# ZhangT-tech/MoCA-Video

Measured on AMD Instinct MI355X. Metric: denoising UNet-steps/sec @16x320x512 fp16, higher is better.
Workload: dtype f16

## Files before the change

### include/moca_hip.h

```cpp
#ifndef MOCA_HIP_H
#define MOCA_HIP_H

#include <stdint.h>

#ifdef __cplusplus
extern "C" {
#endif

#define MOCA_OK            0
#define MOCA_E_BADARG     -1
#define MOCA_E_LAUNCH     -2
#define MOCA_E_NODEVICE   -3
#define MOCA_E_GRAPH      -4

#define MOCA_A_LINEAR   0
#define MOCA_A_CONV3X3  1
#define MOCA_A_TCONV3   2

#define MOCA_EP_GEGLU   1
#define MOCA_EP_OUT_F32 2
#define MOCA_FORCE_SMALL_TILE 4
#define MOCA_EP_COLSUM 16
#define MOCA_EP_LN     32
#define MOCA_EP_GELU    8
// ... 181 lines not shown
    const float* coef;
    const int32_t* win_start;
    const float* mask;
    const float* mask_sums;
    const int32_t* mask_frame;
    const float* enh;
    const float* cond;
    const float* sam_eff;
    const int32_t* sam_idx;
    float cfg_scale, beta, one_minus_beta, gamma, one_minus_gamma;
    int32_t nW, C, Q, f, HW, wb_from;
} moca_fifo_step_params;
int moca_fifo_step_windows_f32(const moca_fifo_step_params* p, void* stream);
int moca_sam_select_masks_f32(const float* cand, const int32_t* cand_off, const int32_t* ncand, const int64_t* t_rows, float* eff,
                              int32_t* eff_idx, int32_t nW, int32_t f, int32_t HW, void* stream);
int moca_fifo_advance_f32(moca_fifo_state* state, float* queue, const float* newframe, float* emitted, int32_t n_slots,
                          int32_t emit_frame, float* mask, float* mask_sums, int32_t C, int32_t Q, int32_t HW, void* stream);
int moca_fifo_prepare_queue_f32(const float* z, const float* noise, float* queue, const float* coef_z, const float* coef_noise,
                                const int32_t* frame_idx, int32_t BC, int32_t Tz, int32_t Q, int32_t HW, void* stream);
int moca_base_set_timestep(const moca_fifo_state* state, const int64_t* table, int32_t S, int64_t* rows, int32_t n, void* stream);
int moca_base_ddim_step_f32(moca_fifo_state* state, float* x, const float* eps_c, const float* eps_u, const float* noise,
                            float* pred_x0, const float* coef, int32_t S, float cfg_scale, int32_t use_scale, int64_t n, void* stream);
int moca_mask_frame_sums_f32(const float* mask, float* sums, int32_t frames, int32_t HW, void* stream);

int moca_freq_mix_3d_f32(const float* x, const float* noise, const float* lpf, float* out,
                         int32_t C, int32_t T, int32_t H, int32_t W, float* ws, void* stream);
int64_t moca_freq_mix_ws_bytes(int32_t C, int32_t T, int32_t H, int32_t W);
int moca_freq_filter_f32(float* lpf, int32_t T, int32_t H, int32_t W, int32_t type, int32_t n,
                         double d_s, double d_t, void* stream);

int moca_graph_begin(void* stream);
int moca_graph_end(void* stream, void** graph_exec_out);
int moca_graph_launch(void* graph_exec, void* stream);
int moca_graph_destroy(void* graph_exec);
int moca_stream_create(void** stream_out);
int moca_stream_destroy(void* stream);
int moca_stream_sync(void* stream);
int moca_event_create(void** ev_out);
int moca_event_record(void* ev, void* stream);
int moca_event_elapsed_ms(void* ev_start, void* ev_stop, float* ms_out);
int moca_event_destroy(void* ev);

#define MOCA_TUNE_GEMM_W80   0
#define MOCA_TUNE_GEMM_G4    1
#define MOCA_TUNE_GEMM_SQ256 2
#define MOCA_TUNE_GEMM_WIDE  3
#define MOCA_TUNE_GN_SLAB    4
#define MOCA_TUNE_GEMM_G4P   5
#define MOCA_TUNE_GEMM_MF32  6
#define MOCA_TUNE_GEMM_SQP   7
#define MOCA_TUNE_SQP_WALK   8
#define MOCA_TUNE_SLAB_F16   9
#define MOCA_TUNE_GEMM_WS    10
#define MOCA_TUNE_COUNT      11
int moca_set_tuning(int32_t knob, int32_t value);
int moca_debug_clock_sampler(void* buf, int32_t blocks, int32_t nsamples, const int32_t* stop, void* stream);

int moca_device_info(char* name, int32_t len, int32_t* cu_count);
const char* moca_version(void);

#ifdef __cplusplus
}
#endif
#endif
```

### moca_video_amd/csrc/gemm.hip

```cpp
#include "common.h"

namespace {

template <int V> struct int_c { static constexpr int value = V; };
struct yes_t { static constexpr bool value = true; };
struct no_t { static constexpr bool value = false; };

constexpr int BM = 128;
constexpr int BK = 64;
constexpr int MOCA_A_LINEAR2 = 3;
constexpr int ROW_BYTES = BK * 2;

struct Geo {
    int C, inH, inW, outH, outW, stride, up, T, HW;
};

__device__ __forceinline__ void remap_tile_2d(int tiles_m, int tiles_n, int xn, int& tile_m, int& tile_n) {
    const int xm = 8 / xn;
    const int sm = tiles_m / xm, sn = tiles_n / xn;
    const int b = blockIdx.x;
    const int xcd = b & 7, j = b >> 3;
    const int xi = xcd / xn, xj = xcd - xi * xn;
    tile_m = xi * sm + j / sn;
    tile_n = xj * sn + j % sn;
// ... 2537 lines not shown
            float sum = 0.f;
#pragma unroll
            for (int r = 0; r < 4; ++r) {
                const float pv = exp2f((sc[i][r] - mx) * sl2e);
                sum += pv;
                pf[i][r] = (half_t)pv;
            }
            sum = xlane16_sum(sum);
            sum = xlane32_sum(sum);
            inv[i] = 1.0f / sum;
        }
#pragma unroll
        for (int i = 0; i < NPX; ++i) {
            half_t* ob = outp + (int64_t)grow(pixs[i] * 16 + fr) * p.ldo + tile_n * 64;
            const bool live = wave + 8 * i < 20;
#pragma unroll
            for (int dt = 0; dt < 4; ++dt) {
                f32x4 o4 = {0.f, 0.f, 0.f, 0.f};
                o4 = __builtin_amdgcn_mfma_f32_16x16x16f16(vfr[i][dt], pf[i], o4, 0, 0, 0);
                half4v h4;
#pragma unroll
                for (int r = 0; r < 4; ++r) h4[r] = (half_t)(o4[r] * inv[i]);
                if (live) *reinterpret_cast<half4v*>(ob + dt * 16 + 4 * fg) = h4;
            }
        }
    } else if constexpr (SQ) {
        store_fp16_tile<512>(p, smem, pitch, TM, BN, m0, n0, tid);
    } else if constexpr (WIDE) {
        if (p.flags & MOCA_EP_LN) store_fp16_tile_ln(p, smem, reinterpret_cast<float*>(smem + TM * pitch), pitch, m0, tid);
        else if (p.flags & (MOCA_EP_COLSUM | MOCA_EP_GSTAT)) store_fp16_tile_colsum<TM, BN>(p, smem, reinterpret_cast<float*>(smem + TM * pitch), pitch, m0, n0, tile_m, tid);
        else if (p.flags & MOCA_EP_ROWSUM) store_fp16_tile_rowsum<512, BN, 8>(p, smem, pitch, TM, m0, n0, tid);
        else store_fp16_tile<512>(p, smem, pitch, TM, BN, m0, n0, tid);
    } else {
        if (p.flags & (MOCA_EP_COLSUM | MOCA_EP_GSTAT)) store_fp16_tile_colsum<TM, BN>(p, smem, reinterpret_cast<float*>(smem + TM * pitch), pitch, m0, n0, tile_m, tid);
        else if (p.flags & MOCA_EP_ROWSUM) store_fp16_tile_rowsum<512, BN, 4>(p, smem, pitch, TM, m0, n0, tid);
        else store_fp16_tile<512>(p, smem, pitch, TM, BN, m0, n0, tid);
    }
    MOCA_STAMP(5);
    MOCA_STAMP_HW();
#endif
}

__device__ __forceinline__ void lds_wr_f2(unsigned a, f32x2 v) { asm volatile("ds_write_b64 %0, %1" ::"v"(a), "v"(v) : "memory"); }
__device__ __forceinline__ void lds_wr_f1(unsigned a, float v) { asm volatile("ds_write_b32 %0, %1" ::"v"(a), "v"(v) : "memory"); }
__device__ __forceinline__ f32x2 lds_rd_f2(unsigned a) { f32x2 v; asm volatile("ds_read_b64 %0, %1" : "=v"(v) : "v"(a) : "memory"); return v; }
__device__ __forceinline__ f32x4 lds_rd_f4(unsigned a) { f32x4 v; asm volatile("ds_read_b128 %0, %1" : "=v"(v) : "v"(a) : "memory"); return v; }
__device__ __forceinline__ float lds_rd_f1(unsigned a) { float v; asm volatile("ds_read_b32 %0, %1" : "=v"(v) : "v"(a) : "memory"); return v; }
__device__ __forceinline__ void lds_wait() { asm volatile("s_waitcnt lgkmcnt(0)" ::: "memory"); __builtin_amdgcn_sched_barrier(0); }

__device__ __forceinline__ int sqp_perm(int rho) {
    return (rho & ~63) + (g4p_perm(rho & 127) & 63);
}

template <bool GEGLU>
__global__ __launch_bounds__(512, 2) void gemm_sqp_kernel(const moca_gemm_params p) {
#if defined(__HIP_DEVICE_COMPILE__)
#ifndef SEG_WAVE
#define SEG_WAVE 0
#endif
    constexpr int MT = 4, NT = 8, KS = 32, RB = 64, WTM = 64, WTN = 128, TM = 256, BN = 256;
    constexpr int A_BYTES = TM * RB, STAGE = A_BYTES + BN * RB, NS = 5, PPW = 4;
    extern __shared__ __attribute__((aligned(16))) char smem[];

    const int tid = threadIdx.x, lane = tid & 63;
    const int wave = __builtin_amdgcn_readfirstlane(tid >> 6);
    const int wave_m = wave >> 1, wave_n = wave & 1;
    const bool late = wave >= 4;
    const int nper = p.reserved2_;
    if (prefetch_block(p, nper, 512)) return;

    const int tiles_n = p.N / BN, tiles_m = (p.M + TM - 1) / TM;
    const int xcd_n = p.reserved4_ >> 8;
    const int J = nper >> 3;
    int q_base, q_cnt, sub_n, tm_base, tn_base;
    {
        const int x = blockIdx.x & 7;
        if (xcd_n > 1) {
            const int xm = 8 / xcd_n, sm = tiles_m / xm;
            sub_n = tiles_n / xcd_n;
            const int xi = x / xcd_n, xj = x - xi * xcd_n;
            tm_base = xi * sm; tn_base = xj * sub_n;
            q_base = 0; q_cnt = sm * sub_n;
        } else {
            const int ntiles = tiles_m * tiles_n, q = ntiles >> 3, r = ntiles & 7;
            q_base = x < r ? x * (q + 1) : r * (q + 1) + (x - r) * q;
            q_cnt = q + (x < r ? 1 : 0);
            sub_n = tiles_n; tm_base = 0; tn_base = 0;
        }
    }
    auto tile_of = [&](int q, int& tm, int& tn) {
        const int l = q_base + q;
        const int a = l / sub_n;
        tm = tm_base + a; tn = tn_base + (l - a * sub_n);
    };
    int q_cur, q_step, q_end;
    {
        const int j = blockIdx.x >> 3;
        if (p.reserved4_ & 2) {
            q_cur = (int)((int64_t)q_cnt * j / J);
            q_end = (int)((int64_t)q_cnt * (j + 1) / J);
            q_step = 1;
        } else {
            q_cur = j; q_end = q_cnt; q_step = J;
        }
    }
    if (q_cur >= q_end) return;
    const int nk = p.K / 32;

    const int lrow = lane >> 2, pch = lane & 3;
    const int lch = pch ^ ((0x78 >> (2 * ((lrow >> 2) & 3))) & 3);
    const __amdgpu_buffer_rsrc_t rsrc_a = __builtin_amdgcn_make_buffer_rsrc(const_cast<void*>(p.a), 0, OOB_OFF, 0x00020000);
    const __amdgpu_buffer_rsrc_t rsrc_w = __builtin_amdgcn_make_buffer_rsrc(const_cast<void*>(p.w), 0, OOB_OFF, 0x00020000);
    unsigned a_off[2], w_off[2];
    int d_q = q_cur, d_k = 0;
    auto set_dma_tile = [&](int q) {
        int tm, tn;
        tile_of(q, tm, tn);
        const bool any = q < q_end;
#pragma unroll
        for (int g = 0; g < 2; ++g) {
            const int row = tm * TM + (g * 8 + wave) * 16 + lrow;
            a_off[g] = (any && row < p.M) ? (unsigned)(((int64_t)row * p.lda + lch * 8) * 2) : OOB_OFF;
            w_off[g] = any ? (unsigned)(((int64_t)(tn * BN + sqp_perm((g * 8 + wave) * 16 + lrow)) * p.ldw + lch * 8) * 2) : OOB_OFF;
        }
    };
    auto issue_pair = [&](int slot_even, int slot_odd) {
        const unsigned soff = (unsigned)(d_k * KS * 2);
        const lds_ptr se = (lds_ptr)smem + slot_even * STAGE, so = (lds_ptr)smem + slot_odd * STAGE;
#pragma unroll
        for (int g = 0; g < 2; ++g) {
            __builtin_amdgcn_raw_ptr_buffer_load_lds(rsrc_a, se + (g * 8 + wave) * 1024, 16, a_off[g], soff, 0, 0);
            __builtin_amdgcn_raw_ptr_buffer_load_lds(rsrc_a, so + (g * 8 + wave) * 1024, 16, a_off[g], soff + KS * 2, 0, 0);
        }
#pragma unroll
        for (int g = 0; g < 2; ++g) {
            __builtin_amdgcn_raw_ptr_buffer_load_lds(rsrc_w, se + A_BYTES + (g * 8 + wave) * 1024, 16, w_off[g], soff, 0, 0);
            __builtin_amdgcn_raw_ptr_buffer_load_lds(rsrc_w, so + A_BYTES + (g * 8 + wave) * 1024, 16, w_off[g], soff + KS * 2, 0, 0);
        }
        d_k += 2;
        if (d_k >= nk) { d_k = 0; d_q += q_step; set_dma_tile(d_q); }
    };

    const int fr = lane & 15, fg = lane >> 4;
    const int swz = (fg ^ ((0x78 >> (2 * ((fr >> 2) & 3))) & 3)) << 4;
    const int a_off0 = (wave_m * WTM + fr) * RB + swz;
    const int b_off0 = A_BYTES + (wave_n * WTN + fr) * RB + swz;
    f32x4 acc[MT][NT];
    half8v af[2][MT], bf[2][NT];
    auto read_tile = [&](auto set_tag, int slot) {
        constexpr int S = decltype(set_tag)::value;
        const char* cur = smem + slot * STAGE;
#pragma unroll
        for (int r = 0; r < NT; ++r) bf[S][r] = *reinterpret_cast<const half8v*>(cur + b_off0 + r * 1024);
#pragma unroll
        for (int r = 0; r < MT; ++r) af[S][r] = *reinterpret_cast<const half8v*>(cur + a_off0 + r * 1024);
    };

    auto tid_now = [&]() -> int {
        int l;
        asm volatile("v_mbcnt_lo_u32_b32 %0, -1, 0\n\tv_mbcnt_hi_u32_b32 %0, -1, %0" : "=v"(l));
        return wave * 64 + l;
    };
    const bool fold = (p.flags & MOCA_EP_LNFOLD) != 0;
    const float* const dummy = reinterpret_cast<const float*>(p.w);
    constexpr unsigned STAT_SCRATCH = 8192;
    const int stat_floats = 2 + 2 * (fold ? p.lnf_nparts : 0);
    auto stat_dma = [&](int q, unsigned slot_off) {
        int tm, tn;
        tile_of(q < q_end ? q : 0, tm, tn);
        const int t = tid_now();
        const int n = tn * BN + sqp_perm(t);
        const int m = min(tm * TM + t, p.M - 1);
        const lds_ptr area = (lds_ptr)smem + slot_off + STAT_SCRATCH + wave * (22 * 256);
        __builtin_amdgcn_global_load_lds((glb_ptr)(fold ? p.lnf_wsum + n : dummy), area, 4, 0, 0);
        __builtin_amdgcn_global_load_lds((glb_ptr)(p.bias ? p.bias + n : dummy), area + 256, 4, 0, 0);
        if (fold) {
            for (int i = 0; i < p.lnf_nparts; ++i) {
                const float* src = p.lnf_part + ((int64_t)i * p.M + m) * 2;
                __builtin_amdgcn_global_load_lds((glb_ptr)src, area + (2 + 2 * i) * 256, 4, 0, 0);
                __builtin_amdgcn_global_load_lds((glb_ptr)(src + 1), area + (3 + 2 * i) * 256, 4, 0, 0);
            }
        }
    };
    auto stat_read = [&](unsigned slot_off, auto after_tag) -> LnFoldRegs {
        constexpr int after = decltype(after_tag)::value;
        asm volatile("s_waitcnt vmcnt(%0)" ::"n"(after) : "memory");
        __builtin_amdgcn_sched_barrier(0);
        int lane_;
        asm volatile("v_mbcnt_lo_u32_b32 %0, -1, 0\n\tv_mbcnt_hi_u32_b32 %0, -1, %0" : "=v"(lane_));
        const unsigned area = (unsigned)(size_t)((lds_ptr)smem + slot_off + STAT_SCRATCH + wave * (22 * 256)) + 4 * lane_;
        const float ws = lds_rd_f1(area), b = lds_rd_f1(area + 256);
        float s = 0.f, qq = 0.f;
        LnFoldRegs f = {1.f, 0.f, 0.f, 0.f};
        if (fold) {
            for (int i = 0; i < p.lnf_nparts; ++i) {
                const float x = lds_rd_f1(area + (2 + 2 * i) * 256), y = lds_rd_f1(area + (3 + 2 * i) * 256);
                lds_wait();
                s += x; qq += y;
            }
// ... 18 lines not shown
        lf = stat_read((NS - 1) * STAGE, int_c<0>{});
    }
    __builtin_amdgcn_s_barrier();
    set_dma_tile(q_cur);
    issue_pair(0, 1);
    issue_pair(2, 3);
    asm volatile("s_waitcnt vmcnt(%0)" ::"n"(2 * PPW) : "memory");
    __builtin_amdgcn_s_barrier();
    if (late) __builtin_amdgcn_s_barrier();

    const bool nt_out = out_streams(p);
    const half_t* __restrict__ resid = reinterpret_cast<const half_t*>(p.residual);
    const half_t* __restrict__ rowadd = reinterpret_cast<const half_t*>(p.rowadd);
    int s0 = 0;
#ifdef MOCA_STAMPS
    int tile_no = 0;
#endif
    while (true) {
        int tm, tn;
        tile_of(q_cur, tm, tn);
        const int m0 = tm * TM, n0 = tn * BN;
#ifdef MOCA_STAMPS
        const bool stamp_it = tile_no == 3;
        if (stamp_it) { MOCA_STAMP(0); }
#endif
#pragma unroll
        for (int mt = 0; mt < MT; ++mt)
#pragma unroll
            for (int nt = 0; nt < NT; ++nt) acc[mt][nt] = f32x4{0.f, 0.f, 0.f, 0.f};
        for (int i = 0; i < nk; i += 2) {
            const int s1 = s0 + 1 == NS ? 0 : s0 + 1;
            const int sp = s0 == 0 ? NS - 1 : s0 - 1;
#ifdef MOCA_STAMPS
            const bool seg = stamp_it && i == SEG_ITER;
            if (seg) MOCA_STAMP_W(8, SEG_WAVE);
#endif
            read_tile(int_c<0>{}, s0);
            asm volatile("s_waitcnt lgkmcnt(0)" ::: "memory");
            __builtin_amdgcn_sched_barrier(0);
#ifdef MOCA_STAMPS
            if (seg) MOCA_STAMP_W(9, SEG_WAVE);
#endif
            __builtin_amdgcn_s_barrier();
#ifdef MOCA_STAMPS
            if (seg) MOCA_STAMP_W(10, SEG_WAVE);
#endif
            {
                const char* nx = smem + s1 * STAGE;
                __builtin_amdgcn_s_setprio(1);
#pragma unroll
                for (int j = 0; j < MT * NT; ++j) {
                    const int mt = j / NT, nt = j % NT;
                    acc[mt][nt] = __builtin_amdgcn_mfma_f32_16x16x32_f16(bf[0][nt], af[0][mt], acc[mt][nt], 0, 0, 0);
                    if (j % 2 == 0 && j / 2 < MT + NT) {
                        const int r = j / 2;
                        __builtin_amdgcn_sched_barrier(0);
                        if (r < NT) bf[1][r] = *reinterpret_cast<const half8v*>(nx + b_off0 + r * 1024);
                        else af[1][r - NT] = *reinterpret_cast<const half8v*>(nx + a_off0 + (r - NT) * 1024);
                        __builtin_amdgcn_sched_barrier(0);
                    }
                }
                __builtin_amdgcn_s_setprio(0);
            }
            asm volatile("s_waitcnt lgkmcnt(0)" ::: "memory");
            __builtin_amdgcn_sched_barrier(0);
#ifdef MOCA_STAMPS
            if (seg) MOCA_STAMP_W(11, SEG_WAVE);
#endif
            __builtin_amdgcn_s_barrier();
#ifdef MOCA_STAMPS
            if (seg) MOCA_STAMP_W(12, SEG_WAVE);
#endif
            issue_pair(sp, s0);
#ifdef MOCA_STAMPS
            if (seg) MOCA_STAMP_W(13, SEG_WAVE);
#endif
            asm volatile("s_waitcnt vmcnt(%0)" ::"n"(2 * PPW) : "memory");
            __builtin_amdgcn_sched_barrier(0);
#ifdef MOCA_STAMPS
            if (seg) MOCA_STAMP_W(14, SEG_WAVE);
#endif
            __builtin_amdgcn_s_barrier();
#ifdef MOCA_STAMPS
            if (seg) MOCA_STAMP_W(15, SEG_WAVE);
#endif
            __builtin_amdgcn_s_setprio(1);
#pragma unroll
            for (int mt = 0; mt < MT; ++mt)
#pragma unroll
                for (int nt = 0; nt < NT; ++nt)
                    acc[mt][nt] = __builtin_amdgcn_mfma_f32_16x16x32_f16(bf[1][nt], af[1][mt], acc[mt][nt], 0, 0, 0);
            __builtin_amdgcn_s_setprio(0);
            __builtin_amdgcn_sched_barrier(0);
#ifdef MOCA_STAMPS
            if (seg) MOCA_STAMP_W(1, SEG_WAVE);
#endif
            __builtin_amdgcn_s_barrier();
#ifdef MOCA_STAMPS
            if (seg) MOCA_STAMP_W(2, SEG_WAVE);
#endif
            s0 = s1 + 1 == NS ? 0 : s1 + 1;
        }
#ifdef MOCA_STAMPS
        if (stamp_it) MOCA_STAMP(3);
#endif
        if (!late) __builtin_amdgcn_s_barrier();
        const unsigned lst = (unsigned)(size_t)((lds_ptr)smem + (s0 == 0 ? NS - 1 : s0 - 1) * STAGE);
        const unsigned lws = lst + 8 * TM, lbi = lws + 4 * BN;
        if (!late) {
            const int t = tid_now();
            lds_wr_f2(lst + 8 * t, f32x2{lf.rs, lf.rb});
            lds_wr_f1(lws + 4 * t, lf.ws);
            lds_wr_f1(lbi + 4 * t, lf.b);
        }
        lds_wait();
        __builtin_amdgcn_s_barrier();
#ifdef MOCA_STAMPS
        if (stamp_it) MOCA_STAMP(4);
#endif
        f32x2 st[MT];
#pragma unroll
        for (int mt = 0; mt < MT; ++mt) st[mt] = lds_rd_f2(lst + 8 * (wave_m * WTM + mt * 16 + fr));
        const int q_next = q_cur + q_step;
        const unsigned stat_slot = (unsigned)((s0 == 0 ? NS - 1 : s0 - 1) * STAGE);
        if (!late) stat_dma(q_next, stat_slot);
#pragma unroll
        for (int grp = 0; grp < 2; ++grp) {
            f32x4 cw[4], cb[4];
#pragma unroll
            for (int t = 0; t < 4; ++t) {
                cw[t] = lds_rd_f4(lws + 4 * (wave_n * WTN + (grp * 4 + t) * 16 + 4 * fg));
                cb[t] = lds_rd_f4(lbi + 4 * (wave_n * WTN + (grp * 4 + t) * 16 + 4 * fg));
            }
            lds_wait();
#pragma unroll
            for (int mt = 0; mt < MT; ++mt) {
                const int m = m0 + wave_m * WTM + mt * 16 + fr;
                f32x4 v[4];
#pragma unroll
                for (int t = 0; t < 4; ++t) v[t] = st[mt][0] * acc[mt][grp * 4 + t] + (st[mt][1] * cw[t] + cb[t]);
                if constexpr (GEGLU) {
                    half8v h;
#pragma unroll
                    for (int nv = 0; nv < 2; ++nv) {
                        const f32x4 r4 = moca_geglu4(v[nv], v[nv + 2]);
                        h[4 * nv + 0] = (half_t)r4[0]; h[4 * nv + 1] = (half_t)r4[1]; h[4 * nv + 2] = (half_t)r4[2]; h[4 * nv + 3] = (half_t)r4[3];
                    }
                    if (m < p.M) st_out8(reinterpret_cast<half_t*>(p.out) + (int64_t)m * p.ldo + (n0 >> 1) + wave_n * 64 + grp * 32 + 8 * fg, h, nt_out);
                } else {
#pragma unroll
                    for (int hh = 0; hh < 2; ++hh) {
                        const int col = n0 + wave_n * WTN + grp * 64 + hh * 32 + 8 * fg;
                        float o[8];
#pragma unroll
                        for (int r = 0; r < 4; ++r) { o[r] = v[2 * hh][r]; o[4 + r] = v[2 * hh + 1][r]; }
                        if (m < p.M) {
                            if (rowadd) {
                                const half8v e = *reinterpret_cast<const half8v*>(rowadd + (int64_t)(m / p.rowadd_div) * p.ld_rowadd + col);
#pragma unroll
                                for (int r = 0; r < 8; ++r) o[r] = (float)(half_t)o[r] + (float)e[r];
                            }
                            if (resid) {
                                const half8v e = *reinterpret_cast<const half8v*>(resid + (int64_t)m * p.ldr + col);
#pragma unroll
                                for (int r = 0; r < 8; ++r) o[r] = (rowadd ? o[r] : (float)(half_t)o[r]) + (float)e[r];
                            }
                            half8v h;
#pragma unroll
                            for (int r = 0; r < 8; ++r) h[r] = (half_t)o[r];
                            st_out8(reinterpret_cast<half_t*>(p.out) + (int64_t)m * p.ldo + col, h, nt_out);
                        }
                    }
                }
            }
        }
#ifdef MOCA_STAMPS
        if (stamp_it) { MOCA_STAMP(5); MOCA_STAMP_HW(); }
        ++tile_no;
#endif
        if (!late) {
            if (m0 + TM > p.M) lf = stat_read(stat_slot, int_c<0>{});
            else lf = stat_read(stat_slot, int_c<(GEGLU ? 8 : 16)>{});
        }
        if (q_next >= q_end) break;
        q_cur = q_next;
        if (late) __builtin_amdgcn_s_barrier();
    }
    asm volatile("s_waitcnt vmcnt(0) lgkmcnt(0)" ::: "memory");
#endif
}

static int choose_xcd_n(const moca_gemm_params& p, int tiles_m, int tiles_n, int TM, int BN) {
    if (p.splits != 1 || p.a_mode != MOCA_A_LINEAR) return 1;
    const double Wtot = (double)p.N * p.K * 2, Atot = (double)p.M * p.K * 2;
    auto cost = [&](int xn) {
        const int xm = 8 / xn;
        const double wsub = (double)(tiles_n / xn) * BN * p.K * 2;
        return (wsub <= 3.6e6 ? xm * Wtot : tiles_m * Wtot) + xn * Atot;
    };
    double best = cost(1);
    int best_xn = 1;
    for (int xn = 2; xn <= 8; xn *= 2) {
        if (tiles_m % (8 / xn) || tiles_n % xn) continue;
        const double c = cost(xn);
        if (c < 0.8 * best) { best = c; best_xn = xn; }
    }
    (void)TM;
    return best_xn;
}

template <int AMODE, int SHAPE>
int launch_gemm_w80s(const moca_gemm_params& p, hipStream_t st) {
    constexpr int TM = SHAPE == 2 ? 256 : (SHAPE == 1 ? 160 : 320), BN = SHAPE == 2 ? 256 : (SHAPE == 1 ? 320 : (SHAPE == 3 ? 192 : 160));
    const int tiles_m = (p.M + TM - 1) / TM, tiles_n = p.N / BN;
    const int nblk = tiles_m * tiles_n * p.splits;
    moca_gemm_params pl = p;
    pl.reserved4_ = (pl.reserved4_ & 0xff) | ((SHAPE == 3 ? 1 : choose_xcd_n(p, tiles_m, tiles_n, TM, BN)) << 8);
    constexpr int lds = 5 * (TM + BN) * 64;
    static bool attr_set = false;
    if (!attr_set) {
        if (hipFuncSetAttribute(reinterpret_cast<const void*>(&gemm_w80s_kernel<AMODE, SHAPE>), hipFuncAttributeMaxDynamicSharedMemorySize, lds) != hipSuccess)
            return MOCA_E_LAUNCH;
        attr_set = true;
    }
    hipLaunchKernelGGL((gemm_w80s_kernel<AMODE, SHAPE>), dim3(nblk + prefetch_blocks(pl)), dim3(512), lds, st, pl);
    MOCA_CHECK_LAUNCH();
    return MOCA_OK;
}

static inline int64_t a_span_bytes(const moca_gemm_params& p) {
    if (p.a_mode == MOCA_A_LINEAR) return ((int64_t)p.M * p.lda + 64) * 2;
    if (p.a_mode == MOCA_A_CONV3X3) return ((int64_t)(p.M / (p.outH * p.outW)) * p.inH * p.inW * p.C + 64) * 2;
    return ((int64_t)p.M * p.C + 64) * 2;
}
static inline bool buffer_addressable(const moca_gemm_params& p) {
    if (p.a2 && ((int64_t)p.M * p.lda2 + 64) * 2 >= (1ll << 31)) return false;
    return a_span_bytes(p) < (1ll << 31) && (int64_t)p.N * p.ldw * 2 < (1ll << 31);
}

static inline int sq256_mode() { return moca_tuning_get(MOCA_TUNE_GEMM_SQ256); }
static inline bool fast_gather(const moca_gemm_params& p);
// ... 78 lines not shown
}

constexpr int G4P_BLOCKS = 512;
static inline bool g4p_ok(const moca_gemm_params& p) {
    if (p.a_mode != MOCA_A_LINEAR || p.splits != 1 || p.N % 128 || p.K % 64 || !buffer_addressable(p)) return false;
    if (p.flags & ~(MOCA_EP_GEGLU | MOCA_EP_LNFOLD)) return false;
    if ((p.flags & MOCA_EP_GEGLU) && (p.residual || p.rowadd)) return false;
    return ((p.M + 255) / 256) * (p.N / 128) >= G4P_BLOCKS;
}
template <bool GEGLU>
int launch_gemm_g4p(const moca_gemm_params& p, hipStream_t st) {
    constexpr int lds = 3 * (256 + 128) * 64 + (2 * 256 + 2 * 128) * 4;
    static bool attr_set = false;
    if (!attr_set) {
        if (hipFuncSetAttribute(reinterpret_cast<const void*>(&gemm_g4p_kernel<GEGLU>), hipFuncAttributeMaxDynamicSharedMemorySize, lds) != hipSuccess)
            return MOCA_E_LAUNCH;
        attr_set = true;
    }
    moca_gemm_params pl = p;
    pl.reserved2_ = G4P_BLOCKS;
    if (moca_tuning_get(MOCA_TUNE_GEMM_MF32)) {
        static bool attr_set_q = false;
        if (!attr_set_q) {
            if (hipFuncSetAttribute(reinterpret_cast<const void*>(&gemm_g4q_kernel<GEGLU>), hipFuncAttributeMaxDynamicSharedMemorySize, lds) != hipSuccess)
                return MOCA_E_LAUNCH;
            attr_set_q = true;
        }
        hipLaunchKernelGGL((gemm_g4q_kernel<GEGLU>), dim3(G4P_BLOCKS + 2 * prefetch_blocks(pl)), dim3(256), lds, st, pl);
    } else {
        hipLaunchKernelGGL((gemm_g4p_kernel<GEGLU>), dim3(G4P_BLOCKS + 2 * prefetch_blocks(pl)), dim3(256), lds, st, pl);
    }
    MOCA_CHECK_LAUNCH();
    return MOCA_OK;
}

constexpr int SQP_BLOCKS = 256;
static inline bool sqp_ok(const moca_gemm_params& p) {
    if (p.a_mode != MOCA_A_LINEAR || p.splits != 1 || p.N % 256 || p.K % 64 || !buffer_addressable(p)) return false;
    if (p.flags & ~(MOCA_EP_GEGLU | MOCA_EP_LNFOLD)) return false;
    if ((p.flags & MOCA_EP_GEGLU) && (p.residual || p.rowadd)) return false;
    return ((p.M + 255) / 256) * (p.N / 256) >= SQP_BLOCKS;
}
template <bool GEGLU>
int launch_gemm_sqp(const moca_gemm_params& p, hipStream_t st) {
    constexpr int lds = 5 * (256 + 256) * 64;
    static bool attr_set = false;
    if (!attr_set) {
        if (hipFuncSetAttribute(reinterpret_cast<const void*>(&gemm_sqp_kernel<GEGLU>), hipFuncAttributeMaxDynamicSharedMemorySize, lds) != hipSuccess)
            return MOCA_E_LAUNCH;
        attr_set = true;
    }
    moca_gemm_params pl = p;
    pl.reserved2_ = SQP_BLOCKS;
    pl.reserved4_ = (pl.reserved4_ & 0xfd) | (choose_xcd_n(p, (p.M + 255) / 256, p.N / 256, 256, 256) << 8) |
                    (moca_tuning_get(MOCA_TUNE_SQP_WALK) ? 2 : 0);
    hipLaunchKernelGGL((gemm_sqp_kernel<GEGLU>), dim3(SQP_BLOCKS + prefetch_blocks(pl)), dim3(512), lds, st, pl);
    MOCA_CHECK_LAUNCH();
    return MOCA_OK;
}

template <int BN, int AMODE, bool FAST>
int launch_gemm_glds(const moca_gemm_params& p, hipStream_t st) {
    const int tiles_m = (p.M + 255) / 256, tiles_n = p.N / BN;
    const int nblk = tiles_m * tiles_n * p.splits;
    constexpr int lds_pipe = 3 * (256 + BN) * ROW_BYTES;
    constexpr int lds_epi = 256 * BN * 4;
    constexpr int lds = lds_pipe > lds_epi ? lds_pipe : lds_epi;
    static bool attr_set = false;
    if (!attr_set) {
        if (hipFuncSetAttribute(reinterpret_cast<const void*>(&gemm_glds_kernel<BN, AMODE, FAST>),
                                hipFuncAttributeMaxDynamicSharedMemorySize, lds) != hipSuccess)
            return MOCA_E_LAUNCH;
        attr_set = true;
    }
    hipLaunchKernelGGL((gemm_glds_kernel<BN, AMODE, FAST>), dim3(nblk + prefetch_blocks(p)), dim3(512), lds, st, p);
    MOCA_CHECK_LAUNCH();
    return MOCA_OK;
}

template <int BN, int AMODE>
int launch_gemm(const moca_gemm_params& p, hipStream_t st) {
    const int tiles_m = (p.M + BM - 1) / BM, tiles_n = p.N / BN;
    const int nblk = tiles_m * tiles_n * p.splits;
    constexpr int lds_pipe = 2 * (BM + BN) * ROW_BYTES;
    constexpr int lds_epi = BM * BN * 4;
    constexpr int lds = lds_pipe > lds_epi ? lds_pipe : lds_epi;
    static bool attr_set = false;
    if (!attr_set) {
        if (hipFuncSetAttribute(reinterpret_cast<const void*>(&gemm_f16_kernel<BN, AMODE>),
                                hipFuncAttributeMaxDynamicSharedMemorySize, lds) != hipSuccess)
            return MOCA_E_LAUNCH;
        attr_set = true;
    }
    hipLaunchKernelGGL((gemm_f16_kernel<BN, AMODE>), dim3(nblk), dim3(256), lds, st, p);
    MOCA_CHECK_LAUNCH();
    return MOCA_OK;
}

}

static void normalise_splits(moca_gemm_params& p) {
    if (p.splits < 1) p.splits = 1;
    if (p.splits > (p.K + BK - 1) / BK) p.splits = (p.K + BK - 1) / BK;
    if (p.splits > 1) {
        const int nkt = (p.K + BK - 1) / BK, kts = (nkt + p.splits - 1) / p.splits;
        p.splits = (nkt + kts - 1) / kts;
    }
}
// ... 295 lines not shown
```

### moca_video_amd/csrc/runtime.hip

```cpp
#include "common.h"
#include <string.h>
#include <stdio.h>
#include <stdlib.h>

extern "C" int moca_graph_begin(void* stream) {
    if (hipStreamBeginCapture(moca_stream(stream), hipStreamCaptureModeThreadLocal) != hipSuccess) return MOCA_E_GRAPH;
    return MOCA_OK;
}

extern "C" int moca_graph_end(void* stream, void** graph_exec_out) {
    if (!graph_exec_out) return MOCA_E_BADARG;
    hipGraph_t g = nullptr;
    if (hipStreamEndCapture(moca_stream(stream), &g) != hipSuccess || !g) return MOCA_E_GRAPH;
    hipGraphExec_t ge = nullptr;
    hipError_t e = hipGraphInstantiate(&ge, g, nullptr, nullptr, 0);
    (void)hipGraphDestroy(g);
    if (e != hipSuccess || !ge) return MOCA_E_GRAPH;
    *graph_exec_out = reinterpret_cast<void*>(ge);
    return MOCA_OK;
}

extern "C" int moca_graph_launch(void* graph_exec, void* stream) {
    if (!graph_exec) return MOCA_E_BADARG;
    if (hipGraphLaunch(reinterpret_cast<hipGraphExec_t>(graph_exec), moca_stream(stream)) != hipSuccess) return MOCA_E_GRAPH;
// ... 45 lines not shown
    int dev = 0;
    if (hipGetDevice(&dev) != hipSuccess) return MOCA_E_NODEVICE;
    hipDeviceProp_t prop;
    if (hipGetDeviceProperties(&prop, dev) != hipSuccess) return MOCA_E_NODEVICE;
    if (name && len > 0) {
        strncpy(name, prop.gcnArchName, (size_t)len - 1);
        name[len - 1] = 0;
    }
    if (cu_count) *cu_count = prop.multiProcessorCount;
    return MOCA_OK;
}

__global__ __launch_bounds__(256) void zero_kernel(uint4* __restrict__ p, int64_t n16, unsigned char* __restrict__ tail, int ntail) {
    for (int64_t i = (int64_t)blockIdx.x * 256 + threadIdx.x; i < n16; i += (int64_t)gridDim.x * 256) p[i] = uint4{0u, 0u, 0u, 0u};
    if (blockIdx.x == 0 && (int)threadIdx.x < ntail) tail[threadIdx.x] = 0;
}

extern "C" int moca_memset_zero(void* ptr, int64_t bytes, void* stream) {
    if (!ptr || bytes < 0 || (reinterpret_cast<uintptr_t>(ptr) & 15)) return MOCA_E_BADARG;
    if (bytes == 0) return MOCA_OK;
    const int64_t n16 = bytes / 16;
    int blocks = (int)((n16 + 255) / 256);
    if (blocks < 1) blocks = 1;
    if (blocks > 1024) blocks = 1024;
    hipLaunchKernelGGL(zero_kernel, dim3(blocks), dim3(256), 0, moca_stream(stream), reinterpret_cast<uint4*>(ptr), n16,
                       reinterpret_cast<unsigned char*>(ptr) + n16 * 16, (int)(bytes - n16 * 16));
    MOCA_CHECK_LAUNCH();
    return MOCA_OK;
}

__global__ __launch_bounds__(64) void clock_sampler_kernel(unsigned long long* __restrict__ buf, int nsamples, const volatile int* stop) {
#if defined(__HIP_DEVICE_COMPILE__)
    if (threadIdx.x) return;
    unsigned long long* b = buf + (size_t)blockIdx.x * nsamples * 2;
    for (int i = 0; i < nsamples; ++i) {
        unsigned long long t, r;
        asm volatile("s_memtime %0\n\ts_memrealtime %1\n\ts_waitcnt lgkmcnt(0)" : "=s"(t), "=s"(r)::"memory");
        b[2 * i] = t;
        b[2 * i + 1] = r;
        if (stop && *stop) break;
        __builtin_amdgcn_s_sleep(127);
        __builtin_amdgcn_s_sleep(127);
    }
#endif
}
extern "C" int moca_debug_clock_sampler(void* buf, int32_t blocks, int32_t nsamples, const int32_t* stop, void* stream) {
    if (!buf || blocks < 1 || blocks > 64 || nsamples < 1 || nsamples > (1 << 20)) return MOCA_E_BADARG;
    hipLaunchKernelGGL(clock_sampler_kernel, dim3(blocks), dim3(64), 0, moca_stream(stream), reinterpret_cast<unsigned long long*>(buf), nsamples,
                       reinterpret_cast<const volatile int*>(stop));
    MOCA_CHECK_LAUNCH();
    return MOCA_OK;
}

static int g_tuning[MOCA_TUNE_COUNT] = {1, 1, 1, 1, 1, 1, 0, 1, 0, 0, 1};
int moca_tuning_get(int knob) { return (knob >= 0 && knob < MOCA_TUNE_COUNT) ? g_tuning[knob] : 0; }
extern "C" int moca_set_tuning(int32_t knob, int32_t value) {
    if (knob < 0 || knob >= MOCA_TUNE_COUNT || value < 0 || value > 2) return MOCA_E_BADARG;
    const int old = g_tuning[knob];
    g_tuning[knob] = value;
    return old;
}
```

### moca_video_amd/lib.py

```python
from __future__ import annotations

import ctypes as C
import os

import torch

_HERE = os.path.dirname(os.path.abspath(__file__))
LIB_PATH = os.environ.get("MOCA_HIP_LIB") or os.path.join(_HERE, "libmoca_hip.so")

MOCA_A_LINEAR, MOCA_A_CONV3X3, MOCA_A_TCONV3 = 0, 1, 2
MOCA_EP_GEGLU, MOCA_EP_OUT_F32, MOCA_FORCE_SMALL_TILE, MOCA_EP_GELU, MOCA_EP_COLSUM, MOCA_EP_LN = 1, 2, 4, 8, 16, 32
MOCA_EP_ROWSUM, MOCA_EP_LNFOLD, MOCA_EP_GSTAT, MOCA_EP_TATTN, MOCA_EP_SLABS = 64, 128, 256, 512, 1024
MOCA_TUNE_GEMM_W80, MOCA_TUNE_GEMM_G4, MOCA_TUNE_GEMM_SQ256, MOCA_TUNE_GEMM_WIDE, MOCA_TUNE_GN_SLAB, MOCA_TUNE_GEMM_G4P, MOCA_TUNE_GEMM_MF32, MOCA_TUNE_GEMM_SQP, MOCA_TUNE_SQP_WALK = 0, 1, 2, 3, 4, 5, 6, 7, 8
MOCA_TUNE_SLAB_F16 = 9
MOCA_TUNE_GEMM_WS = 10

_ERR = {0: "ok", -1: "bad argument (shape/alignment contract)", -2: "HIP launch/runtime error",
        -3: "no gfx950 device", -4: "graph capture/replay failed"}


class MocaHipError(RuntimeError):
    pass


class GemmParams(C.Structure):
    _fields_ = [
        ("a", C.c_void_p), ("w", C.c_void_p), ("out", C.c_void_p), ("bias", C.c_void_p),
        ("rowadd", C.c_void_p), ("residual", C.c_void_p), ("splitk_ws", C.c_void_p),
        ("M", C.c_int32), ("N", C.c_int32), ("K", C.c_int32),
        ("lda", C.c_int32), ("ldw", C.c_int32), ("ldo", C.c_int32), ("ldr", C.c_int32), ("ld_rowadd", C.c_int32),
        ("rowadd_div", C.c_int32), ("a_mode", C.c_int32), ("C", C.c_int32),
        ("inH", C.c_int32), ("inW", C.c_int32), ("outH", C.c_int32), ("outW", C.c_int32),
        ("stride", C.c_int32), ("up", C.c_int32), ("T", C.c_int32), ("HW", C.c_int32),
        ("flags", C.c_int32), ("splits", C.c_int32), ("nopad_lo", C.c_int32), ("prefetch_kib", C.c_int32),
        ("colsum", C.c_void_p), ("ln_gamma", C.c_void_p), ("ln_beta", C.c_void_p), ("ln_out", C.c_void_p),
        ("ld_ln", C.c_int32), ("ln_eps", C.c_float),
        ("rowsum", C.c_void_p), ("lnf_part", C.c_void_p), ("lnf_wsum", C.c_void_p),
        ("lnf_nparts", C.c_int32), ("reserved2_", C.c_int32),
        ("gstat", C.c_void_p), ("gstat_rows", C.c_int32), ("tattn_scale", C.c_float),
        ("prefetch", C.c_void_p), ("up_phase", C.c_int32), ("reserved4_", C.c_int32),
        ("a2", C.c_void_p), ("lda2", C.c_int32), ("k1", C.c_int32), ("gstat_cpg", C.c_int32), ("gstat_coff", C.c_int32),
        ("wgroup_rows", C.c_int32), ("wgroup_stride", C.c_int32),
    ]


class FifoState(C.Structure):
    _fields_ = [("head", C.c_int32), ("iter", C.c_int32), ("seed_lo", C.c_uint32), ("seed_hi", C.c_uint32),
                ("ext_noise", C.c_int32), ("reserved_", C.c_int32 * 3)]


class FifoStepParams(C.Structure):
    _fields_ = [
        ("state", C.c_void_p), ("x", C.c_void_p), ("eps_c", C.c_void_p), ("eps_u", C.c_void_p), ("noise", C.c_void_p),
        ("momentum", C.c_void_p), ("queue", C.c_void_p), ("x_prev", C.c_void_p), ("pred_x0", C.c_void_p), ("coef", C.c_void_p),
        ("win_start", C.c_void_p), ("mask", C.c_void_p), ("mask_sums", C.c_void_p), ("mask_frame", C.c_void_p),
        ("enh", C.c_void_p), ("cond", C.c_void_p), ("sam_eff", C.c_void_p), ("sam_idx", C.c_void_p),
        ("cfg_scale", C.c_float), ("beta", C.c_float), ("one_minus_beta", C.c_float), ("gamma", C.c_float),
        ("one_minus_gamma", C.c_float),
        ("nW", C.c_int32), ("C", C.c_int32), ("Q", C.c_int32), ("f", C.c_int32), ("HW", C.c_int32), ("wb_from", C.c_int32),
    ]


_vp, _i32, _i64, _f32, _f64 = C.c_void_p, C.c_int32, C.c_int64, C.c_float, C.c_double
SIGNATURES = {
    "moca_gemm_f16": (C.c_int, [C.POINTER(GemmParams), _vp]),
    "moca_gemm_splitk_ws_bytes": (_i64, [_i32, _i32, _i32]),
    "moca_gemm_colsum_rows": (C.c_int, [C.POINTER(GemmParams)]),
    "moca_gemm_ln_ok": (C.c_int, [C.POINTER(GemmParams)]),
# ... 125 lines not shown
```

Measured before the change: 60.46.

## Split tail-wave SQP GEMM tiles into half or quarter sub-tiles across idle blocks

The persistent SQP GEMM kernel body moves into a templated sqp_walk helper parameterised by the per-wave MT/NT fragment counts. When the per-XCD tile count leaves a small remainder relative to the blocks per XCD, those leftover 256x256 tiles are split into N-halves or quarters and spread across the otherwise idle blocks. This targets the tail-wave imbalance of the final round. In exchange, each sub-tile reloads the full A panel and covers less MFMA work per LDS stage. The path is gated by a new tuning knob that defaults on and applies only when the round count is at most 16.

```diff
diff --git a/include/moca_hip.h b/include/moca_hip.h
--- a/include/moca_hip.h
+++ b/include/moca_hip.h
@@ -257,7 +257,8 @@
 #define MOCA_TUNE_SQP_WALK   8
 #define MOCA_TUNE_SLAB_F16   9
 #define MOCA_TUNE_GEMM_WS    10
-#define MOCA_TUNE_COUNT      11
+#define MOCA_TUNE_SQP_TAIL   11
+#define MOCA_TUNE_COUNT      12
 int moca_set_tuning(int32_t knob, int32_t value);
 int moca_debug_clock_sampler(void* buf, int32_t blocks, int32_t nsamples, const int32_t* stop, void* stream);
 
diff --git a/moca_video_amd/csrc/gemm.hip b/moca_video_amd/csrc/gemm.hip
--- a/moca_video_amd/csrc/gemm.hip
+++ b/moca_video_amd/csrc/gemm.hip
@@ -2613,90 +2613,66 @@
     return (rho & ~63) + (g4p_perm(rho & 127) & 63);
 }
 
-template <bool GEGLU>
-__global__ __launch_bounds__(512, 2) void gemm_sqp_kernel(const moca_gemm_params p) {
+struct SqpSet { int q_base, sub_n, tm_base, tn_base; };
+
+template <bool GEGLU, int MT, int NT>
+__device__ __forceinline__ void sqp_walk(const moca_gemm_params& p, char* smem, const int tid, const SqpSet set, int q_cur, const int q_end,
+                                         const int q_step, const int mh, const int nh) {
 #if defined(__HIP_DEVICE_COMPILE__)
 #ifndef SEG_WAVE
 #define SEG_WAVE 0
 #endif
-    constexpr int MT = 4, NT = 8, KS = 32, RB = 64, WTM = 64, WTN = 128, TM = 256, BN = 256;
-    constexpr int A_BYTES = TM * RB, STAGE = A_BYTES + BN * RB, NS = 5, PPW = 4;
-    extern __shared__ __attribute__((aligned(16))) char smem[];
-
-    const int tid = threadIdx.x, lane = tid & 63;
+    constexpr int KS = 32, RB = 64, WTM = 64, WTN = 128, TM = 256, BN = 256;
+    constexpr int A_BYTES = TM * RB, STAGE = A_BYTES + BN * RB, NS = 5;
+    constexpr int NAG = MT / 2, NWG = NT / 4, PPW = NAG + NWG;
+    static_assert((MT == 4 || MT == 2) && (NT == 8 || NT == 4), "whole tile, N half or quarter");
+
+    const int lane = tid & 63;
     const int wave = __builtin_amdgcn_readfirstlane(tid >> 6);
     const int wave_m = wave >> 1, wave_n = wave & 1;
     const bool late = wave >= 4;
-    const int nper = p.reserved2_;
-    if (prefetch_block(p, nper, 512)) return;
-
-    const int tiles_n = p.N / BN, tiles_m = (p.M + TM - 1) / TM;
-    const int xcd_n = p.reserved4_ >> 8;
-    const int J = nper >> 3;
-    int q_base, q_cnt, sub_n, tm_base, tn_base;
-    {
-        const int x = blockIdx.x & 7;
-        if (xcd_n > 1) {
-            const int xm = 8 / xcd_n, sm = tiles_m / xm;
-            sub_n = tiles_n / xcd_n;
-            const int xi = x / xcd_n, xj = x - xi * xcd_n;
-            tm_base = xi * sm; tn_base = xj * sub_n;
-            q_base = 0; q_cnt = sm * sub_n;
-        } else {
-            const int ntiles = tiles_m * tiles_n, q = ntiles >> 3, r = ntiles & 7;
-            q_base = x < r ? x * (q + 1) : r * (q + 1) + (x - r) * q;
-            q_cnt = q + (x < r ? 1 : 0);
-            sub_n = tiles_n; tm_base = 0; tn_base = 0;
-        }
-    }
+    const int row_sub = MT == 4 ? 0 : mh * 32;
+    const int col_sub = NT == 8 ? 0 : nh * 64;
     auto tile_of = [&](int q, int& tm, int& tn) {
-        const int l = q_base + q;
-        const int a = l / sub_n;
-        tm = tm_base + a; tn = tn_base + (l - a * sub_n);
+        const int l = set.q_base + q;
+        const int a = l / set.sub_n;
+        tm = set.tm_base + a; tn = set.tn_base + (l - a * set.sub_n);
     };
-    int q_cur, q_step, q_end;
-    {
-        const int j = blockIdx.x >> 3;
-        if (p.reserved4_ & 2) {
-            q_cur = (int)((int64_t)q_cnt * j / J);
-            q_end = (int)((int64_t)q_cnt * (j + 1) / J);
-            q_step = 1;
-        } else {
-            q_cur = j; q_end = q_cnt; q_step = J;
-        }
-    }
-    if (q_cur >= q_end) return;
     const int nk = p.K / 32;
 
+    auto a_piece = [&](int g) { const int i = g * 8 + wave; return MT == 4 ? i : ((i >> 1) << 2) + mh * 2 + (i & 1); };
+    auto w_piece = [&](int g) { const int i = g * 8 + wave; return NT == 8 ? i : ((i >> 2) << 3) + nh * 4 + (i & 3); };
     const int lrow = lane >> 2, pch = lane & 3;
     const int lch = pch ^ ((0x78 >> (2 * ((lrow >> 2) & 3))) & 3);
     const __amdgpu_buffer_rsrc_t rsrc_a = __builtin_amdgcn_make_buffer_rsrc(const_cast<void*>(p.a), 0, OOB_OFF, 0x00020000);
     const __amdgpu_buffer_rsrc_t rsrc_w = __builtin_amdgcn_make_buffer_rsrc(const_cast<void*>(p.w), 0, OOB_OFF, 0x00020000);
-    unsigned a_off[2], w_off[2];
+    unsigned a_off[NAG], w_off[NWG];
     int d_q = q_cur, d_k = 0;
     auto set_dma_tile = [&](int q) {
         int tm, tn;
         tile_of(q, tm, tn);
         const bool any = q < q_end;
 #pragma unroll
-        for (int g = 0; g < 2; ++g) {
-            const int row = tm * TM + (g * 8 + wave) * 16 + lrow;
+        for (int g = 0; g < NAG; ++g) {
+            const int row = tm * TM + a_piece(g) * 16 + lrow;
             a_off[g] = (any && row < p.M) ? (unsigned)(((int64_t)row * p.lda + lch * 8) * 2) : OOB_OFF;
-            w_off[g] = any ? (unsigned)(((int64_t)(tn * BN + sqp_perm((g * 8 + wave) * 16 + lrow)) * p.ldw + lch * 8) * 2) : OOB_OFF;
-        }
+        }
+#pragma unroll
+        for (int g = 0; g < NWG; ++g)
+            w_off[g] = any ? (unsigned)(((int64_t)(tn * BN + sqp_perm(w_piece(g) * 16 + lrow)) * p.ldw + lch * 8) * 2) : OOB_OFF;
     };
     auto issue_pair = [&](int slot_even, int slot_odd) {
         const unsigned soff = (unsigned)(d_k * KS * 2);
         const lds_ptr se = (lds_ptr)smem + slot_even * STAGE, so = (lds_ptr)smem + slot_odd * STAGE;
 #pragma unroll
-        for (int g = 0; g < 2; ++g) {
-            __builtin_amdgcn_raw_ptr_buffer_load_lds(rsrc_a, se + (g * 8 + wave) * 1024, 16, a_off[g], soff, 0, 0);
-            __builtin_amdgcn_raw_ptr_buffer_load_lds(rsrc_a, so + (g * 8 + wave) * 1024, 16, a_off[g], soff + KS * 2, 0, 0);
-        }
-#pragma unroll
-        for (int g = 0; g < 2; ++g) {
-            __builtin_amdgcn_raw_ptr_buffer_load_lds(rsrc_w, se + A_BYTES + (g * 8 + wave) * 1024, 16, w_off[g], soff, 0, 0);
-            __builtin_amdgcn_raw_ptr_buffer_load_lds(rsrc_w, so + A_BYTES + (g * 8 + wave) * 1024, 16, w_off[g], soff + KS * 2, 0, 0);
+        for (int g = 0; g < NAG; ++g) {
+            __builtin_amdgcn_raw_ptr_buffer_load_lds(rsrc_a, se + a_piece(g) * 1024, 16, a_off[g], soff, 0, 0);
+            __builtin_amdgcn_raw_ptr_buffer_load_lds(rsrc_a, so + a_piece(g) * 1024, 16, a_off[g], soff + KS * 2, 0, 0);
+        }
+#pragma unroll
+        for (int g = 0; g < NWG; ++g) {
+            __builtin_amdgcn_raw_ptr_buffer_load_lds(rsrc_w, se + A_BYTES + w_piece(g) * 1024, 16, w_off[g], soff, 0, 0);
+            __builtin_amdgcn_raw_ptr_buffer_load_lds(rsrc_w, so + A_BYTES + w_piece(g) * 1024, 16, w_off[g], soff + KS * 2, 0, 0);
         }
         d_k += 2;
         if (d_k >= nk) { d_k = 0; d_q += q_step; set_dma_tile(d_q); }
@@ -2704,8 +2680,8 @@
 
     const int fr = lane & 15, fg = lane >> 4;
     const int swz = (fg ^ ((0x78 >> (2 * ((fr >> 2) & 3))) & 3)) << 4;
-    const int a_off0 = (wave_m * WTM + fr) * RB + swz;
-    const int b_off0 = A_BYTES + (wave_n * WTN + fr) * RB + swz;
+    const int a_off0 = (wave_m * WTM + row_sub + fr) * RB + swz;
+    const int b_off0 = A_BYTES + (wave_n * WTN + col_sub + fr) * RB + swz;
     f32x4 acc[MT][NT];
     half8v af[2][MT], bf[2][NT];
     auto read_tile = [&](auto set_tag, int slot) {
@@ -2830,8 +2806,9 @@
                 for (int j = 0; j < MT * NT; ++j) {
                     const int mt = j / NT, nt = j % NT;
                     acc[mt][nt] = __builtin_amdgcn_mfma_f32_16x16x32_f16(bf[0][nt], af[0][mt], acc[mt][nt], 0, 0, 0);
-                    if (j % 2 == 0 && j / 2 < MT + NT) {
-                        const int r = j / 2;
+                    constexpr int RS = MT * NT >= 2 * (MT + NT) ? 2 : 1;
+                    if (j % RS == 0 && j / RS < MT + NT) {
+                        const int r = j / RS;
                         __builtin_amdgcn_sched_barrier(0);
                         if (r < NT) bf[1][r] = *reinterpret_cast<const half8v*>(nx + b_off0 + r * 1024);
                         else af[1][r - NT] = *reinterpret_cast<const half8v*>(nx + a_off0 + (r - NT) * 1024);
@@ -2898,12 +2875,13 @@
 #endif
         f32x2 st[MT];
 #pragma unroll
-        for (int mt = 0; mt < MT; ++mt) st[mt] = lds_rd_f2(lst + 8 * (wave_m * WTM + mt * 16 + fr));
+        for (int mt = 0; mt < MT; ++mt) st[mt] = lds_rd_f2(lst + 8 * (wave_m * WTM + row_sub + mt * 16 + fr));
         const int q_next = q_cur + q_step;
         const unsigned stat_slot = (unsigned)((s0 == 0 ? NS - 1 : s0 - 1) * STAGE);
         if (!late) stat_dma(q_next, stat_slot);
 #pragma unroll
-        for (int grp = 0; grp < 2; ++grp) {
+        for (int gi = 0; gi < NT / 4; ++gi) {
+            const int grp = NT == 8 ? gi : nh;
             f32x4 cw[4], cb[4];
 #pragma unroll
             for (int t = 0; t < 4; ++t) {
@@ -2913,10 +2891,10 @@
             lds_wait();
 #pragma unroll
             for (int mt = 0; mt < MT; ++mt) {
-                const int m = m0 + wave_m * WTM + mt * 16 + fr;
+                const int m = m0 + wave_m * WTM + row_sub + mt * 16 + fr;
                 f32x4 v[4];
 #pragma unroll
-                for (int t = 0; t < 4; ++t) v[t] = st[mt][0] * acc[mt][grp * 4 + t] + (st[mt][1] * cw[t] + cb[t]);
+                for (int t = 0; t < 4; ++t) v[t] = st[mt][0] * acc[mt][gi * 4 + t] + (st[mt][1] * cw[t] + cb[t]);
                 if constexpr (GEGLU) {
                     half8v h;
 #pragma unroll
@@ -2958,13 +2936,69 @@
 #endif
         if (!late) {
             if (m0 + TM > p.M) lf = stat_read(stat_slot, int_c<0>{});
-            else lf = stat_read(stat_slot, int_c<(GEGLU ? 8 : 16)>{});
+            else lf = stat_read(stat_slot, int_c<(MT * (NT / 4) * (GEGLU ? 1 : 2))>{});
         }
         if (q_next >= q_end) break;
         q_cur = q_next;
         if (late) __builtin_amdgcn_s_barrier();
     }
     asm volatile("s_waitcnt vmcnt(0) lgkmcnt(0)" ::: "memory");
+#endif
+}
+
+template <bool GEGLU>
+__global__ __launch_bounds__(512, 2) void gemm_sqp_kernel(const moca_gemm_params p) {
+#if defined(__HIP_DEVICE_COMPILE__)
+    constexpr int TM = 256, BN = 256;
+    extern __shared__ __attribute__((aligned(16))) char smem[];
+    const int nper = p.reserved2_;
+    if (prefetch_block(p, nper, 512)) return;
+
+    const int tiles_n = p.N / BN, tiles_m = (p.M + TM - 1) / TM;
+    const int xcd_n = p.reserved4_ >> 8;
+    const int J = nper >> 3;
+    SqpSet set;
+    int q_cnt;
+    {
+        const int x = blockIdx.x & 7;
+        if (xcd_n > 1) {
+            const int xm = 8 / xcd_n, sm = tiles_m / xm;
+            set.sub_n = tiles_n / xcd_n;
+            const int xi = x / xcd_n, xj = x - xi * xcd_n;
+            set.tm_base = xi * sm; set.tn_base = xj * set.sub_n;
+            set.q_base = 0; q_cnt = sm * set.sub_n;
+        } else {
+            const int ntiles = tiles_m * tiles_n, q = ntiles >> 3, r = ntiles & 7;
+            set.q_base = x < r ? x * (q + 1) : r * (q + 1) + (x - r) * q;
+            q_cnt = q + (x < r ? 1 : 0);
+            set.sub_n = tiles_n; set.tm_base = 0; set.tn_base = 0;
+        }
+    }
+    const int j = blockIdx.x >> 3;
+    const int wave_s = __builtin_amdgcn_readfirstlane(threadIdx.x >> 6);
+    int q_whole = q_cnt, cut = 0;
+    if (p.reserved4_ & 8) {
+        const int left = q_cnt % J;
+        cut = left == 0 ? 0 : (left * 4 <= J ? 2 : (left * 2 <= J ? 1 : 0));
+        if (cut) q_whole = q_cnt - left;
+    }
+    int q_cur, q_step, q_end;
+    if (p.reserved4_ & 2) {
+        q_cur = (int)((int64_t)q_whole * j / J);
+        q_end = (int)((int64_t)q_whole * (j + 1) / J);
+        q_step = 1;
+    } else {
+        q_cur = j; q_end = q_whole; q_step = J;
+    }
+    if (q_cur < q_end) sqp_walk<GEGLU, 4, 8>(p, smem, threadIdx.x, set, q_cur, q_end, q_step, 0, 0);
+    if (cut == 0 || j >= ((q_cnt - q_whole) << cut)) return;
+    __builtin_amdgcn_s_barrier();
+    const int q_sub = q_whole + (j >> cut), part = j & ((1 << cut) - 1);
+    int lane2;
+    asm volatile("v_mbcnt_lo_u32_b32 %0, -1, 0\n\tv_mbcnt_hi_u32_b32 %0, -1, %0" : "=v"(lane2));
+    const int tid2 = wave_s * 64 + lane2;
+    if (cut == 1) sqp_walk<GEGLU, 4, 4>(p, smem, tid2, set, q_sub, q_sub + 1, 1, 0, part);
+    else sqp_walk<GEGLU, 2, 4>(p, smem, tid2, set, q_sub, q_sub + 1, 1, part >> 1, part & 1);
 #endif
 }
 
@@ -3149,8 +3183,9 @@
     }
     moca_gemm_params pl = p;
     pl.reserved2_ = SQP_BLOCKS;
-    pl.reserved4_ = (pl.reserved4_ & 0xfd) | (choose_xcd_n(p, (p.M + 255) / 256, p.N / 256, 256, 256) << 8) |
-                    (moca_tuning_get(MOCA_TUNE_SQP_WALK) ? 2 : 0);
+    const int rounds = (((p.M + 255) / 256) * (p.N / 256) / 8 + SQP_BLOCKS / 8 - 1) / (SQP_BLOCKS / 8);
+    pl.reserved4_ = (pl.reserved4_ & 0xf5) | (choose_xcd_n(p, (p.M + 255) / 256, p.N / 256, 256, 256) << 8) |
+                    (moca_tuning_get(MOCA_TUNE_SQP_WALK) ? 2 : 0) | ((moca_tuning_get(MOCA_TUNE_SQP_TAIL) && rounds <= 16) ? 8 : 0);
     hipLaunchKernelGGL((gemm_sqp_kernel<GEGLU>), dim3(SQP_BLOCKS + prefetch_blocks(pl)), dim3(512), lds, st, pl);
     MOCA_CHECK_LAUNCH();
     return MOCA_OK;
diff --git a/moca_video_amd/csrc/runtime.hip b/moca_video_amd/csrc/runtime.hip
--- a/moca_video_amd/csrc/runtime.hip
+++ b/moca_video_amd/csrc/runtime.hip
@@ -121,7 +121,7 @@
     return MOCA_OK;
 }
 
-static int g_tuning[MOCA_TUNE_COUNT] = {1, 1, 1, 1, 1, 1, 0, 1, 0, 0, 1};
+static int g_tuning[MOCA_TUNE_COUNT] = {1, 1, 1, 1, 1, 1, 0, 1, 0, 0, 1, 1};
 int moca_tuning_get(int knob) { return (knob >= 0 && knob < MOCA_TUNE_COUNT) ? g_tuning[knob] : 0; }
 extern "C" int moca_set_tuning(int32_t knob, int32_t value) {
     if (knob < 0 || knob >= MOCA_TUNE_COUNT || value < 0 || value > 2) return MOCA_E_BADARG;
diff --git a/moca_video_amd/lib.py b/moca_video_amd/lib.py
--- a/moca_video_amd/lib.py
+++ b/moca_video_amd/lib.py
@@ -14,6 +14,7 @@
 MOCA_TUNE_GEMM_W80, MOCA_TUNE_GEMM_G4, MOCA_TUNE_GEMM_SQ256, MOCA_TUNE_GEMM_WIDE, MOCA_TUNE_GN_SLAB, MOCA_TUNE_GEMM_G4P, MOCA_TUNE_GEMM_MF32, MOCA_TUNE_GEMM_SQP, MOCA_TUNE_SQP_WALK = 0, 1, 2, 3, 4, 5, 6, 7, 8
 MOCA_TUNE_SLAB_F16 = 9
 MOCA_TUNE_GEMM_WS = 10
+MOCA_TUNE_SQP_TAIL = 11
 
 _ERR = {0: "ok", -1: "bad argument (shape/alignment contract)", -2: "HIP launch/runtime error",
         -3: "no gfx950 device", -4: "graph capture/replay failed"}
```

Result: no change. 60.71 (median of 6 runs) (+0.4%).
